# GuidoManni/BodySLAM

Hardware: AMD Instinct MI355X
Metric: frames/sec depth+pose+back-proj, 640x480 seq (higher is better)
Workload: dtype f16

## Files before the change

### bodyslam_amd/_lib.py

```python
from __future__ import annotations

import ctypes as C
import os
from typing import Optional

import torch

_HERE = os.path.dirname(os.path.abspath(__file__))
LIB_PATH = os.environ.get("BODYSLAM_HIP_LIB") or os.path.join(_HERE, "libbodyslam_hip.so")

F32, F16, BF16 = 0, 1, 2
F64 = 3
ACT_NONE, ACT_RELU, ACT_GELU, ACT_SOFTPLUS, ACT_SOFTPLUS_FAST = 0, 1, 2, 3, 4
OUT_PLAIN, OUT_SHUFFLE, OUT_QKV = 0, 1, 2

_TORCH2BS = {torch.float32: F32, torch.float16: F16, torch.bfloat16: BF16}
BS2TORCH = {F32: torch.float32, F16: torch.float16, BF16: torch.bfloat16}


class BodySlamHipError(RuntimeError):
    pass


class GemmDesc(C.Structure):
# ... 476 lines not shown
def cast(x, out):
    check(load_library().bs_cast(p(x), p(out), x.numel(), dt(out), stream_ptr()), "bs_cast")


def cast_split(x, out, rows, cols, f8=False):
    check(load_library().bs_cast_split(p(x), p(out), rows, cols, dt(out) | (32 if f8 else 0), stream_ptr()), "bs_cast_split")


def relu_split(x, out, rows, cols, f8=False):
    check(load_library().bs_relu_split(p(x), p(out), rows, cols, dt(out) | (32 if f8 else 0), stream_ptr()), "bs_relu_split")


def preprocess_patches(frames, out, B, H, W, nh, nw, flip):
    check(load_library().bs_preprocess_patches(p(frames), p(out), B, H, W, nh, nw, int(flip), dt(out), stream_ptr()),
          "bs_preprocess_patches")


def preprocess_image(frames, out, B, H, W, nh, nw, flip):
    check(load_library().bs_preprocess_image(p(frames), p(out), B, H, W, nh, nw, int(flip), stream_ptr()), "bs_preprocess_image")


def fill_rows(x, v, B, rows_per_image, cols):
    check(load_library().bs_fill_rows(p(x), p(v), B, rows_per_image, cols, stream_ptr()), "bs_fill_rows")


def resize_bilinear_nhwc(x, out, B, Hin, Win, Cch, Hout, Wout, align_corners=True, split=False):
    check(load_library().bs_resize_bilinear_nhwc(p(x), p(out), B, Hin, Win, Cch, Hout, Wout, int(align_corners) | (4 if split == 2 else (2 if split else 0)), dt(x),
                                                 stream_ptr()), "bs_resize_bilinear_nhwc")


def depth_u16_to_m(depth_u16: torch.Tensor, depth_scale: float, depth_trunc: float) -> torch.Tensor:
    assert depth_u16.dtype == torch.int16 and depth_u16.is_cuda and depth_u16.is_contiguous()
    out = torch.empty(depth_u16.shape, dtype=torch.float32, device=depth_u16.device)
    check(load_library().bs_depth_u16_to_m(p(depth_u16), depth_u16.numel(), float(depth_scale), float(depth_trunc), p(out), stream_ptr()),
          "bs_depth_u16_to_m")
    return out


def col_mean(A, lda, row0, rows_per_group, groups, row_step, K, out, zero=None):
    assert out.dtype == torch.bfloat16 and (zero is None or zero.dtype == torch.float32)
    check(load_library().bs_col_mean(p(A), lda, row0, rows_per_group, groups, row_step, K, p(out), p(zero), 0 if zero is None else zero.numel(),
                                     dt(A), stream_ptr()), "bs_col_mean")


def rank1_bias(abar, dw, out):
    assert abar.dtype == torch.bfloat16 and dw.dtype == torch.bfloat16 and out.dtype == torch.float32
    G, K = abar.shape
    N = dw.shape[0]
    assert dw.shape[1] == K and tuple(out.shape) == (G, N)
    check(load_library().bs_rank1_bias(p(abar), p(dw), p(out), G, N, K, stream_ptr()), "bs_rank1_bias")


def upconv_tapsum(y, bias, out, B, Hin, Win, Cout, Hout, Wout, align_corners=True, split=False, relu=True):
    check(load_library().bs_upconv_tapsum(p(y), p(bias), p(out), B, Hin, Win, Cout, Hout, Wout,
                                          int(align_corners) | (4 if split == 2 else (2 if split else 0)), int(relu), dt(out), stream_ptr()),
          "bs_upconv_tapsum")


def upconv_fused(x, w, bias, out, B, Hin, Win, Cin, Cout, mode=0, split=0, relu=True, f8_scales=(127, 127, 127, 127)):
    check(load_library().bs_upconv_fused(p(x), p(w), p(bias), p(out), B, Hin, Win, Cin, Cout, 2 * Hin, 2 * Win,
                                         1 | (4 if split == 2 else (2 if split else 0)), int(relu), mode, *[int(v) for v in f8_scales], dt(out),
                                         stream_ptr()), "bs_upconv_fused")


def resize_bias_relu_nhwc(x, bias, out, B, Hin, Win, Cch, Hout, Wout, split=False):
    check(load_library().bs_resize_bias_relu_nhwc(p(x), p(bias), p(out), B, Hin, Win, Cch, Hout, Wout, 1 | (2 if split else 0), dt(out), stream_ptr()),
          "bs_resize_bias_relu_nhwc")


def attractor_step(A, bins_prev, bins_out, route, B, Hp, Wp, H, W, groups, n_bins, n_attr):
    check(load_library().bs_attractor_step(p(A), p(bins_prev), p(bins_out), p(route), B, Hp, Wp, H, W, groups, n_bins, n_attr,
                                           stream_ptr()), "bs_attractor_step")


def mlp2(x, ldx, W1, b1, W2, b2, out, M, K1, N1, N2, act2=ACT_SOFTPLUS_FAST):
    check(load_library().bs_mlp2(p(x), ldx, p(W1), p(b1), p(W2), p(b2), p(out), M, K1, N1, N2, act2, dt(x), stream_ptr()), "bs_mlp2")


def mlp2_add(emb, prev, W1, b1, W2, b2, out, B, Hp, Wp, H, W, K1, N1, N2, act2=ACT_SOFTPLUS_FAST, split=False):
    check(load_library().bs_mlp2_add(p(emb), p(prev), p(W1), p(b1), p(W2), p(b2), p(out), B, Hp, Wp, H, W, K1, N1, N2, act2,
                                     dt(emb) | (16 if split else 0), stream_ptr()), "bs_mlp2_add")


def projector_level(z, b_c1, emb_prev, Wc2, b_c2, We, b_e, x_out, emb_out, eh_out, B, Hl, Wl, H, W, PM, E, NE):
    check(load_library().bs_projector_level(p(z), p(b_c1), p(emb_prev), p(Wc2), p(b_c2), p(We), p(b_e), p(x_out), p(emb_out), p(eh_out), B, Hl, Wl,
                                            H, W, PM, E, NE, dt(z), stream_ptr()), "bs_projector_level")


def add_resized(x, prev, out, B, Hp, Wp, H, W, Cch, split=False):
    check(load_library().bs_add_resized(p(x), p(prev), p(out), B, Hp, Wp, H, W, Cch, dt(x) | (16 if split else 0), stream_ptr()),
          "bs_add_resized")


def logbinom_depth(last, Eh, bins, w0_last, w2, b2, route, depth, B, H, W, He, We, min_temp, max_temp):
    check(load_library().bs_logbinom_depth(p(last), p(Eh), p(bins), p(w0_last), p(w2), p(b2), p(route), p(depth), B, H, W, He, We,
                                           min_temp, max_temp, dt(last), stream_ptr()), "bs_logbinom_depth")


def small_attention(qkv, out, B, S, nheads):
    check(load_library().bs_small_attention(p(qkv), p(out), B, S, nheads, dt(out), stream_ptr()), "bs_small_attention")


def route_argmax(logits, ld, route, B):
    check(load_library().bs_route_argmax(p(logits), ld, p(route), B, stream_ptr()), "bs_route_argmax")


def postprocess_depth(depth_net, depth_m, depth_u16, B, H, W, nh, nw, flip):
    check(load_library().bs_postprocess_depth(p(depth_net), p(depth_m), p(depth_u16), B, H, W, nh, nw, int(flip), stream_ptr()),
          "bs_postprocess_depth")


def cyclepose_im2col(frames, pairs, out, P, H, W):
    check(load_library().bs_cyclepose_im2col(p(frames), p(pairs), p(out), P, H, W, dt(out), stream_ptr()), "bs_cyclepose_im2col")


def instnorm_relu_nhwc(x, out, out_f32, scratch, P, HW, Cch, eps=1e-5):
    check(load_library().bs_instnorm_relu_nhwc(p(x), p(out), p(out_f32), p(scratch), P, HW, Cch, eps, dt(out), stream_ptr()),
          "bs_instnorm_relu_nhwc")


def avgpool_nhwc(x, out, P, HW, Cch):
    check(load_library().bs_avgpool_nhwc(p(x), p(out), P, HW, Cch, stream_ptr()), "bs_avgpool_nhwc")


def cyclepose_head(pooled, x2, w_skip_pool, w_skip_x2, b_skip, w1, b1, w2, b2, pose7, T, scratch, P, HW, Cch):
    check(load_library().bs_cyclepose_head(p(pooled), p(x2), p(w_skip_pool), p(w_skip_x2), p(b_skip), p(w1), p(b1), p(w2), p(b2),
                                           p(pose7), p(T), p(scratch), P, HW, Cch, stream_ptr()), "bs_cyclepose_head")


def backproject(depth_u16, K4, depth_scale, depth_trunc, poses, xyz, idx, count, scratch, B, H, W):
    Karr = (C.c_double * 4)(*[float(v) for v in K4])
    check(load_library().bs_backproject(p(depth_u16), B, H, W, C.cast(Karr, C.c_void_p), float(depth_scale), float(depth_trunc),
                                        p(poses), p(xyz), p(idx), p(count), p(scratch), stream_ptr()), "bs_backproject")


def pose_chain(t_rel, N, g0, g_abs):
    g0arr = None
    if g0 is not None:
        g0arr = C.cast((C.c_double * 16)(*[float(v) for v in g0]), C.c_void_p)
    check(load_library().bs_pose_chain(p(t_rel), N, g0arr, p(g_abs), stream_ptr()), "bs_pose_chain")


def pose_chain_from(t_rel, N, g0_dev, g_abs):
    check(load_library().bs_pose_chain_from(p(t_rel), N, p(g0_dev), p(g_abs), stream_ptr()), "bs_pose_chain_from")


def pixel_to_3d(uvd, K4, out, n):
    Karr = (C.c_double * 4)(*[float(v) for v in K4])
    check(load_library().bs_pixel_to_3d(p(uvd), n, C.cast(Karr, C.c_void_p), p(out), stream_ptr()), "bs_pixel_to_3d")


DEPTH_SCALE_MEDIAN, DEPTH_SCALE_FIXED = 0, 1
DEPTH_METRICS_FIELDS = 16


def depth_metrics(pred, gt, gt_lo, gt_hi, scale, workspace, out):
    B, H, W = pred.shape
    assert tuple(gt.shape) == (B, H, W) and pred.is_contiguous() and gt.is_contiguous()
    assert out.dtype == torch.float64 and tuple(out.shape) == (B, DEPTH_METRICS_FIELDS) and out.is_contiguous()
    mode = DEPTH_SCALE_MEDIAN if scale is None else DEPTH_SCALE_FIXED
    check(load_library().bs_depth_metrics(p(pred), p(gt), B, H, W, float(gt_lo), float(gt_hi), mode, 0.0 if scale is None else float(scale),
                                          p(workspace), workspace.numel() * workspace.element_size(), p(out), stream_ptr()), "bs_depth_metrics")


def depth_metrics_workspace(B: int, H: int, W: int) -> int:
    return int(load_library().bs_depth_metrics_workspace(B, H, W))


TRAJ_EVO, TRAJ_TRAINING = 0, 1
# ... 24 lines not shown
```

### bodyslam_amd/csrc/mlp2.hip

```cpp
#include "common.h"

namespace bs {

constexpr int MLP_BM = 256, MLP_K1 = 128, MLP_N1 = 256, MLP_LDS = 131072;

struct MlpAddGeom {
    const void* prev;
    int Hp, Wp, H, W;
    float sy, sx;
};

template <typename T, int FUSE, int SPLIT>
__global__ __launch_bounds__(512) void mlp2_kernel(const T* __restrict__ x, int ldx, const T* __restrict__ W1, const float* __restrict__ b1,
                                                   const T* __restrict__ W2, const float* __restrict__ b2, float* __restrict__ out, int M, int N2,
                                                   int act2, MlpAddGeom ag) {
    typedef typename T16<T>::v8 v8;
    typedef typename T16<T>::v4 v4;
    extern __shared__ __attribute__((aligned(16))) char smem[];
    const int tid = threadIdx.x, lane = tid & 63;
    const int wave = __builtin_amdgcn_readfirstlane(tid >> 6);
    const int m0 = blockIdx.x * MLP_BM;
    const int frow = lane & 15, fq = lane >> 4;

    {
        const int r8 = lane >> 3, chunk = (lane & 7) ^ r8;
        const bool whole = m0 + MLP_BM <= M;
        const char* xl = reinterpret_cast<const char*>(x + (int64_t)(m0 + r8) * ldx + chunk * 8);
        const char* wl = reinterpret_cast<const char*>(W1 + (int64_t)r8 * MLP_K1 + chunk * 8);
        const int64_t xstep = (int64_t)8 * ldx * 2;
#pragma unroll
        for (int it = 0; it < 4; ++it) {
            const int rg = wave + it * 8;
            const char* xs = xl + rg * xstep;
            if (!whole) {
                int m = m0 + rg * 8 + r8;
                m = m < M ? m : M - 1;
                xs = reinterpret_cast<const char*>(x + (int64_t)m * ldx + chunk * 8);
            }
#pragma unroll
            for (int seg = 0; seg < 2; ++seg) {
                if (!FUSE) glds16(xs + seg * 128, smem + seg * 32768 + rg * 1024);
                glds16(wl + (int64_t)rg * 8 * MLP_K1 * 2 + seg * 128, smem + 65536 + seg * 32768 + rg * 1024);
            }
        }
    }
    if constexpr (FUSE) {
        const T* prev = reinterpret_cast<const T*>(ag.prev);
        constexpr int C = MLP_K1, PS = SPLIT ? 2 : 1;
        auto ld8 = [&](const T* ptr, float (&dst)[8]) {
            const v8 h = *reinterpret_cast<const v8*>(ptr);
#pragma unroll
            for (int e = 0; e < 8; ++e) dst[e] = (float)h[e];
            if (SPLIT) {
                const v8 l = *reinterpret_cast<const v8*>(ptr + C);
#pragma unroll
                for (int e = 0; e < 8; ++e) dst[e] += (float)l[e];
            }
        };
        typedef int i32x4_ __attribute__((ext_vector_type(4)));
        i32x4_* rtab = reinterpret_cast<i32x4_*>(smem + MLP_LDS);
        if (tid < MLP_BM) {
            int m = m0 + tid;
            m = m < M ? m : M - 1;
            const int hw = ag.H * ag.W;
            const int b = m / hw, rem = m - b * hw;
            const int oy = rem / ag.W, ox = rem - oy * ag.W;
            const float fy = ag.sy * (float)oy, fx = ag.sx * (float)ox;
            int y0 = (int)fy, x0 = (int)fx;
            y0 = y0 > ag.Hp - 1 ? ag.Hp - 1 : y0;
            x0 = x0 > ag.Wp - 1 ? ag.Wp - 1 : x0;
            const int y1 = y0 + (y0 < ag.Hp - 1 ? 1 : 0), x1 = x0 + (x0 < ag.Wp - 1 ? 1 : 0);
            const float ly = fy - (float)y0, lx = fx - (float)x0, hy = 1.0f - ly, hx = 1.0f - lx;
            const int pb0 = b * ag.Hp * ag.Wp;
            rtab[2 * tid] = i32x4_{(pb0 + y0 * ag.Wp + x0) * C * PS, (pb0 + y0 * ag.Wp + x1) * C * PS, (pb0 + y1 * ag.Wp + x0) * C * PS,
                                   (pb0 + y1 * ag.Wp + x1) * C * PS};
            rtab[2 * tid + 1] = i32x4_{__float_as_int(hx), __float_as_int(lx), __float_as_int(hy), __float_as_int(ly)};
        }
        __syncthreads();
#pragma unroll 2
        for (int k = 0; k < MLP_BM * 16 / 512; ++k) {
            const int idx = tid + k * 512, r = idx >> 4, c8 = idx & 15;
            int m = m0 + r;
            m = m < M ? m : M - 1;
            const i32x4_ po = rtab[2 * r], pw = rtab[2 * r + 1];
            const float hx = __int_as_float(pw[0]), lx = __int_as_float(pw[1]), hy = __int_as_float(pw[2]), ly = __int_as_float(pw[3]);
            const T* pb = prev + c8 * 8;
            float q00[8], q01[8], q10[8], q11[8], av[8];
            ld8(pb + po[0], q00);
            ld8(pb + po[1], q01);
            ld8(pb + po[2], q10);
            ld8(pb + po[3], q11);
            ld8(x + (int64_t)m * ldx + c8 * 8, av);
            const f32x2_ hx2 = {hx, hx}, lx2 = {lx, lx}, hy2 = {hy, hy}, ly2 = {ly, ly};
            v8 o;
#pragma unroll
            for (int e = 0; e < 8; e += 2) {
                f32x2_ v = bilerp2(f32x2_{q00[e], q00[e + 1]}, f32x2_{q01[e], q01[e + 1]}, f32x2_{q10[e], q10[e + 1]}, f32x2_{q11[e], q11[e + 1]}, hx2, lx2,
                                   hy2, ly2);
                v += f32x2_{av[e], av[e + 1]};
                o[e] = T16<T>::from_f32(v[0]);
                o[e + 1] = T16<T>::from_f32(v[1]);
            }
            *reinterpret_cast<v8*>(smem + (c8 >> 3) * 32768 + r * 128 + (((c8 & 7) ^ (r & 7)) << 4)) = o;
        }
    }
    asm volatile("s_waitcnt vmcnt(0)" ::: "memory");
    __syncthreads();

    const int wr = wave >> 1, wc = wave & 1;
    f32x4 acc1[4][8];
#pragma unroll
    for (int i = 0; i < 4; ++i)
#pragma unroll
        for (int j = 0; j < 8; ++j) acc1[i][j] = f32x4{0.f, 0.f, 0.f, 0.f};
    const int sw = frow & 7;
#pragma unroll
    for (int ks = 0; ks < 4; ++ks) {
        const int seg = ks >> 1, kc = (ks & 1) * 4;
        const int coff = ((kc + fq) ^ sw) << 4;
        v8 xf[4], wf[8];
#pragma unroll
        for (int i = 0; i < 4; ++i) xf[i] = *reinterpret_cast<const v8*>(smem + seg * 32768 + (wr * 64 + i * 16 + frow) * 128 + coff);
#pragma unroll
        for (int j = 0; j < 8; ++j) wf[j] = *reinterpret_cast<const v8*>(smem + 65536 + seg * 32768 + (wc * 128 + j * 16 + frow) * 128 + coff);
#pragma unroll
        for (int i = 0; i < 4; ++i)
#pragma unroll
            for (int j = 0; j < 8; ++j) acc1[i][j] = T16<T>::mfma16(wf[j], xf[i], acc1[i][j]);
    }
    const int NF2 = (N2 + 15) >> 4;
    v8 w2f[2][8];
#pragma unroll
    for (int j = 0; j < 2; ++j)
#pragma unroll
        for (int ks = 0; ks < 8; ++ks) {
            const int n = j * 16 + frow;
            v8 z;
#pragma unroll
            for (int e = 0; e < 8; ++e) z[e] = T16<T>::from_f32(0.f);
            w2f[j][ks] = (j < NF2 && n < N2) ? *reinterpret_cast<const v8*>(W2 + (int64_t)n * MLP_N1 + ks * 32 + fq * 8) : z;
        }
    __syncthreads();
#pragma unroll
    for (int j = 0; j < 8; ++j) {
        const int n = wc * 128 + j * 16 + fq * 4;
        const f32x4 bb = *reinterpret_cast<const f32x4*>(b1 + n);
        const int seg = n >> 6, chunk = (n & 63) >> 3, sub = (n & 7) * 2;
#pragma unroll
        for (int i = 0; i < 4; ++i) {
            const int m = wr * 64 + i * 16 + frow;
            v4 h;
#pragma unroll
            for (int e = 0; e < 4; ++e) h[e] = T16<T>::from_f32(fmaxf(acc1[i][j][e] + bb[e], 0.0f));
            *reinterpret_cast<v4*>(smem + seg * 32768 + m * 128 + ((chunk ^ (m & 7)) << 4) + sub) = h;
        }
    }
    __syncthreads();

    f32x4 acc2[2][2];
#pragma unroll
    for (int i = 0; i < 2; ++i)
#pragma unroll
        for (int j = 0; j < 2; ++j) acc2[i][j] = f32x4{0.f, 0.f, 0.f, 0.f};
#pragma unroll
    for (int ks = 0; ks < 8; ++ks) {
        const int seg = ks >> 1, kc = (ks & 1) * 4;
        const int coff = ((kc + fq) ^ sw) << 4;
        v8 af[2];
#pragma unroll
        for (int i = 0; i < 2; ++i) af[i] = *reinterpret_cast<const v8*>(smem + seg * 32768 + (wave * 32 + i * 16 + frow) * 128 + coff);
#pragma unroll
        for (int i = 0; i < 2; ++i)
#pragma unroll
            for (int j = 0; j < 2; ++j)
                if (j < NF2) acc2[i][j] = T16<T>::mfma16(w2f[j][ks], af[i], acc2[i][j]);
    }
#pragma unroll
    for (int j = 0; j < 2; ++j) {
        const int n = j * 16 + fq * 4;
        if (j >= NF2 || n >= N2) continue;
        const f32x4 bb = *reinterpret_cast<const f32x4*>(b2 + n);
#pragma unroll
        for (int i = 0; i < 2; ++i) {
            const int m = m0 + wave * 32 + i * 16 + frow;
            if (m >= M) continue;
            f32x4 y;
#pragma unroll
            for (int e = 0; e < 4; ++e) y[e] = apply_act(acc2[i][j][e] + bb[e], act2);
            *reinterpret_cast<f32x4*>(out + (int64_t)m * N2 + n) = y;
        }
    }
}

template <typename T, int FUSE, int SPLIT>
static int launch_mlp2(const void* x, int ldx, const void* W1, const float* b1, const void* W2, const float* b2, float* out, int M, int N2, int act2,
                       const MlpAddGeom& ag, hipStream_t st) {
    BS_MAX_DYNAMIC_LDS(((const void*)mlp2_kernel<T, FUSE, SPLIT>), MLP_LDS + (FUSE ? MLP_BM * 32 : 0));
    hipLaunchKernelGGL((mlp2_kernel<T, FUSE, SPLIT>), dim3(cdiv(M, MLP_BM)), dim3(512), MLP_LDS + (FUSE ? MLP_BM * 32 : 0), st, (const T*)x, ldx, (const T*)W1, b1, (const T*)W2, b2,
                       out, M, N2, act2, ag);
    BS_CHECK_LAUNCH();
    return BS_OK;
}

static int mlp2_check(const char* who, const void* x, const void* W1, const float* b1, const void* W2, const float* b2, float* out, int M, int K1,
                      int N1, int N2, int act2, int dtype) {
    if (!initialized()) { set_error("%s: call bs_init first", who); return BS_ERR_NOT_INIT; }
    BS_REQUIRE(x && W1 && b1 && W2 && b2 && out, "%s: null operand", who);
    BS_REQUIRE(dtype == BS_F16 || dtype == BS_BF16, "%s: dtype must be f16 or bf16", who);
    BS_REQUIRE(K1 == MLP_K1 && N1 == MLP_N1, "%s: built for K1 = %d, N1 = %d (got %d, %d)", who, MLP_K1, MLP_N1, K1, N1);
    BS_REQUIRE(N2 > 0 && N2 <= 32 && N2 % 4 == 0, "%s: N2 = %d must be a multiple of 4 in 4 .. 32", who, N2);
    BS_REQUIRE(M > 0, "%s: M = %d", who, M);
    BS_REQUIRE(act2 == BS_ACT_NONE || act2 == BS_ACT_RELU || act2 == BS_ACT_SOFTPLUS || act2 == BS_ACT_SOFTPLUS_FAST || act2 == BS_ACT_GELU, "%s: unknown activation %d", who, act2);
    return BS_OK;
}

}

extern "C" int bs_mlp2(const void* x, int32_t ldx, const void* W1, const float* b1, const void* W2, const float* b2, float* out, int32_t M,
                       int32_t K1, int32_t N1, int32_t N2, int32_t act2, int32_t dtype, void* stream) {
    using namespace bs;
    const int rc = mlp2_check("bs_mlp2", x, W1, b1, W2, b2, out, M, K1, N1, N2, act2, dtype);
    if (rc != BS_OK) return rc;
    BS_REQUIRE(ldx >= K1 && ldx % 8 == 0, "bs_mlp2: ldx = %d (rows of >= K1 16-bit values, 16-byte aligned)", ldx);
    hipStream_t st = (hipStream_t)stream;
    const MlpAddGeom ag{};
    return dtype == BS_F16 ? launch_mlp2<f16, 0, 0>(x, ldx, W1, b1, W2, b2, out, M, N2, act2, ag, st)
                           : launch_mlp2<bf16, 0, 0>(x, ldx, W1, b1, W2, b2, out, M, N2, act2, ag, st);
}

extern "C" int bs_mlp2_add(const void* emb, const void* prev, const void* W1, const float* b1, const void* W2, const float* b2, float* out,
                           int32_t B, int32_t Hp, int32_t Wp, int32_t H, int32_t W, int32_t K1, int32_t N1, int32_t N2, int32_t act2, int32_t dtype,
                           void* stream) {
    using namespace bs;
    const int split = (dtype & 16) ? 1 : 0;
    dtype &= 15;
    BS_REQUIRE(B > 0 && Hp > 0 && Wp > 0 && H > 0 && W > 0 && (int64_t)B * H * W < 0x7FFFFFFFll, "bs_mlp2_add: bad geometry");
    const int M = B * H * W;
    const int rc = mlp2_check("bs_mlp2_add", emb, W1, b1, W2, b2, out, M, K1, N1, N2, act2, dtype);
    if (rc != BS_OK) return rc;
    BS_REQUIRE(prev, "bs_mlp2_add: null operand");
    BS_REQUIRE((int64_t)B * Hp * Wp * K1 * (split ? 2 : 1) < 0x7FFFFFFFll, "bs_mlp2_add: prev too large for 32-bit element offsets");
    MlpAddGeom ag;
    ag.prev = prev; ag.Hp = Hp; ag.Wp = Wp; ag.H = H; ag.W = W;
    ag.sy = H > 1 ? (float)(Hp - 1) / (float)(H - 1) : 0.f;
    ag.sx = W > 1 ? (float)(Wp - 1) / (float)(W - 1) : 0.f;
    const int ldx = K1 * (split ? 2 : 1);
    hipStream_t st = (hipStream_t)stream;
    if (dtype == BS_F16)
        return split ? launch_mlp2<f16, 1, 1>(emb, ldx, W1, b1, W2, b2, out, M, N2, act2, ag, st)
                     : launch_mlp2<f16, 1, 0>(emb, ldx, W1, b1, W2, b2, out, M, N2, act2, ag, st);
    return split ? launch_mlp2<bf16, 1, 1>(emb, ldx, W1, b1, W2, b2, out, M, N2, act2, ag, st)
                 : launch_mlp2<bf16, 1, 0>(emb, ldx, W1, b1, W2, b2, out, M, N2, act2, ag, st);
}
```

### bodyslam_amd/csrc/projector.hip

```cpp
#include "common.h"

namespace bs {

constexpr int PL_PM = 64, PL_E = 128, PL_NE_MAX = 80;
constexpr int PL_WE_OFF = 2 * PL_E * 128;
constexpr int PL_W_BYTES = PL_WE_OFF + 2 * PL_NE_MAX * 128;
constexpr int PL_SLICE = 8192, PL_LDS = PL_W_BYTES + 8 * PL_SLICE;

struct PlArgs {
    const void *z, *prev, *Wc2, *We;
    const float *b1, *bc2, *be;
    void *x_out, *emb_out;
    float* eh_out;
    int B, Hl, Wl, H, W, NE;
    float sy, sx;
    int nslices;
};

#define PL_MFMA_FENCE()                                    \
    do {                                                   \
        __builtin_amdgcn_sched_barrier(0);                 \
        asm volatile("s_nop 15\n\ts_nop 15" ::: "memory"); \
        __builtin_amdgcn_sched_barrier(0);                 \
    } while (0)

template <typename T>
__global__ __launch_bounds__(512) void projector_level_kernel(PlArgs a) {
    typedef typename T16<T>::v8 v8;
    extern __shared__ __attribute__((aligned(16))) char smem[];
    const int tid = threadIdx.x, lane = tid & 63;
    const int wave = __builtin_amdgcn_readfirstlane(tid >> 6);
    const int frow = lane & 15, fq = lane >> 4, sw = frow & 7;
    const int c8 = lane & 7, pq = lane >> 3;
    const int NE = a.NE, nje = NE >> 4;

    {
        const int r8 = lane >> 3, chunk = (lane & 7) ^ r8;
        const int ngc = PL_E / 8, nge = NE / 8, total = 2 * ngc + (a.We ? 2 * nge : 0);
        for (int g = wave; g < total; g += 8) {
            const T* src;
            char* dst;
            if (g < 2 * ngc) {
                const int part = g / ngc, rg = g - part * ngc;
                src = reinterpret_cast<const T*>(a.Wc2) + (int64_t)(rg * 8 + r8) * (3 * PL_PM) + part * (2 * PL_PM) + chunk * 8;
                dst = smem + part * (PL_E * 128) + rg * 1024;
            } else {
                const int g2 = g - 2 * ngc, part = g2 / nge, rg = g2 - part * nge;
                src = reinterpret_cast<const T*>(a.We) + (int64_t)(rg * 8 + r8) * (3 * PL_PM) + part * (2 * PL_PM) + chunk * 8;
                dst = smem + PL_WE_OFF + part * (NE * 128) + rg * 1024;
            }
            glds16(src, dst);
        }
        asm volatile("s_waitcnt vmcnt(0)" ::: "memory");
        __syncthreads();
    }

    char* my = smem + PL_W_BYTES + wave * PL_SLICE;
    const T* zp = reinterpret_cast<const T*>(a.z);
    const T* pp = reinterpret_cast<const T*>(a.prev);
    T* xo = reinterpret_cast<T*>(a.x_out);
    T* eo = reinterpret_cast<T*>(a.emb_out);
    float bz[8];
#pragma unroll
    for (int e = 0; e < 8; ++e) bz[e] = a.b1[c8 * 8 + e];

    auto ld8 = [&](const T* ptr, int lo_off, float (&dst)[8]) {
        const v8 h = *reinterpret_cast<const v8*>(ptr);
        const v8 l = *reinterpret_cast<const v8*>(ptr + lo_off);
#pragma unroll
        for (int e = 0; e < 8; ++e) dst[e] = (float)h[e];
#pragma unroll
        for (int e = 0; e < 8; ++e) dst[e] += (float)l[e];
    };

    for (int s = blockIdx.x * 8 + wave; s < a.nslices; s += gridDim.x * 8) {
        const int m0 = s * 32;
        const int row = m0 / a.W, ox0 = m0 - row * a.W;
        const int b = row / a.H, oy = row - b * a.H;
        const float fy = a.sy * (float)oy;
        int y0 = (int)fy;
        y0 = y0 > a.Hl - 1 ? a.Hl - 1 : y0;
        const int y1 = y0 + (y0 < a.Hl - 1 ? 1 : 0);
        const float ly = fy - (float)y0, hy = 1.0f - ly;
        const f32x2_ hy2 = {hy, hy}, ly2 = {ly, ly};
        const int64_t img = (int64_t)b * a.Hl * a.Wl;
        const int r0 = y0 * a.Wl, r1 = y1 * a.Wl;

        const T* zb = zp + img * (2 * PL_PM) + c8 * 8;
#pragma unroll
        for (int it = 0; it < 4; ++it) {
            const int p = it * 8 + pq, ox = ox0 + p;
            const float fx = a.sx * (float)ox;
            int x0 = (int)fx;
            x0 = x0 > a.Wl - 1 ? a.Wl - 1 : x0;
            const int x1 = x0 + (x0 < a.Wl - 1 ? 1 : 0);
            const float lx = fx - (float)x0, hx = 1.0f - lx;
            float q00[8], q01[8], q10[8], q11[8];
            ld8(zb + (int64_t)(r0 + x0) * (2 * PL_PM), PL_PM, q00);
            ld8(zb + (int64_t)(r0 + x1) * (2 * PL_PM), PL_PM, q01);
            ld8(zb + (int64_t)(r1 + x0) * (2 * PL_PM), PL_PM, q10);
            ld8(zb + (int64_t)(r1 + x1) * (2 * PL_PM), PL_PM, q11);
            const f32x2_ hx2 = {hx, hx}, lx2 = {lx, lx};
            v8 o, ol;
#pragma unroll
            for (int e = 0; e < 8; e += 2) {
                f32x2_ v = bilerp2(f32x2_{q00[e], q00[e + 1]}, f32x2_{q01[e], q01[e + 1]}, f32x2_{q10[e], q10[e + 1]}, f32x2_{q11[e], q11[e + 1]}, hx2, lx2,
                                   hy2, ly2);
                v += f32x2_{bz[e], bz[e + 1]};
                v = f32x2_{fmaxf(v[0], 0.0f), fmaxf(v[1], 0.0f)};
#pragma unroll
                for (int u = 0; u < 2; ++u) {
                    o[e + u] = T16<T>::from_f32(v[u]);
                    ol[e + u] = T16<T>::from_f32(v[u] - (float)o[e + u]);
                }
            }
            const int pos = p * 128 + ((c8 ^ (p & 7)) << 4);
            *reinterpret_cast<v8*>(my + pos) = o;
            *reinterpret_cast<v8*>(my + 4096 + pos) = ol;
        }
        asm volatile("s_waitcnt lgkmcnt(0)" ::: "memory");
        __builtin_amdgcn_wave_barrier();

        if (a.eh_out) {
            f32x4 acc[2][PL_NE_MAX / 16];
#pragma unroll
            for (int i = 0; i < 2; ++i)
#pragma unroll
                for (int j = 0; j < PL_NE_MAX / 16; ++j) acc[i][j] = f32x4{0.f, 0.f, 0.f, 0.f};
#pragma unroll
            for (int pass = 0; pass < 3; ++pass) {
                const int aseg = pass == 1 ? 4096 : 0, wpart = pass == 2 ? NE * 128 : 0;
#pragma unroll
                for (int ks = 0; ks < 2; ++ks) {
                    const int coff = ((ks * 4 + fq) ^ sw) << 4;
                    v8 xf[2];
#pragma unroll
                    for (int i = 0; i < 2; ++i) xf[i] = *reinterpret_cast<const v8*>(my + aseg + (i * 16 + frow) * 128 + coff);
#pragma unroll
                    for (int j = 0; j < PL_NE_MAX / 16; ++j) {
                        if (j < nje) {
                            const v8 wf = *reinterpret_cast<const v8*>(smem + PL_WE_OFF + wpart + (j * 16 + frow) * 128 + coff);
#pragma unroll
                            for (int i = 0; i < 2; ++i) acc[i][j] = T16<T>::mfma16(wf, xf[i], acc[i][j]);
                        }
                    }
                }
            }
            PL_MFMA_FENCE();
#pragma unroll
            for (int j = 0; j < PL_NE_MAX / 16; ++j) {
                if (j < nje) {
                    const int n = j * 16 + fq * 4;
                    const f32x4 bb = *reinterpret_cast<const f32x4*>(a.be + n);
#pragma unroll
                    for (int i = 0; i < 2; ++i) {
                        const f32x4 y = acc[i][j] + bb;
                        *reinterpret_cast<f32x4*>(a.eh_out + (int64_t)(m0 + i * 16 + frow) * NE + n) = y;
                    }
                }
            }
        }

        f32x4 acc[2][8];
#pragma unroll
        for (int i = 0; i < 2; ++i)
#pragma unroll
            for (int j = 0; j < 8; ++j) acc[i][j] = f32x4{0.f, 0.f, 0.f, 0.f};
#pragma unroll
        for (int pass = 0; pass < 3; ++pass) {
            const int aseg = pass == 1 ? 4096 : 0, wpart = pass == 2 ? PL_E * 128 : 0;
#pragma unroll
            for (int ks = 0; ks < 2; ++ks) {
                const int coff = ((ks * 4 + fq) ^ sw) << 4;
                v8 xf[2];
#pragma unroll
                for (int i = 0; i < 2; ++i) xf[i] = *reinterpret_cast<const v8*>(my + aseg + (i * 16 + frow) * 128 + coff);
#pragma unroll
                for (int j = 0; j < 8; ++j) {
                    const v8 wf = *reinterpret_cast<const v8*>(smem + wpart + (j * 16 + frow) * 128 + coff);
#pragma unroll
                    for (int i = 0; i < 2; ++i) acc[i][j] = T16<T>::mfma16(wf, xf[i], acc[i][j]);
                }
            }
        }
        PL_MFMA_FENCE();
        asm volatile("s_waitcnt lgkmcnt(0)" ::: "memory");
        __builtin_amdgcn_wave_barrier();

        const T* pb = pp + img * (2 * PL_E) + c8 * 8;
#pragma unroll
        for (int h = 0; h < 2; ++h) {
#pragma unroll
            for (int jj = 0; jj < 4; ++jj) {
                const f32x4 bb = *reinterpret_cast<const f32x4*>(a.bc2 + h * 64 + jj * 16 + fq * 4);
#pragma unroll
                for (int i = 0; i < 2; ++i) {
                    const int m = i * 16 + frow;
                    *reinterpret_cast<f32x4*>(my + m * 256 + (((jj * 4 + fq) ^ frow) << 4)) = acc[i][h * 4 + jj] + bb;
                }
            }
            asm volatile("s_waitcnt lgkmcnt(0)" ::: "memory");
            __builtin_amdgcn_wave_barrier();
#pragma unroll
            for (int it = 0; it < 4; ++it) {
                const int p = it * 8 + pq, ox = ox0 + p;
                const float fx = a.sx * (float)ox;
                int x0 = (int)fx;
                x0 = x0 > a.Wl - 1 ? a.Wl - 1 : x0;
                const int x1 = x0 + (x0 < a.Wl - 1 ? 1 : 0);
                const float lx = fx - (float)x0, hx = 1.0f - lx;
                float q00[8], q01[8], q10[8], q11[8];
                const T* pc = pb + h * 64;
                ld8(pc + (int64_t)(r0 + x0) * (2 * PL_E), PL_E, q00);
                ld8(pc + (int64_t)(r0 + x1) * (2 * PL_E), PL_E, q01);
                ld8(pc + (int64_t)(r1 + x0) * (2 * PL_E), PL_E, q10);
                ld8(pc + (int64_t)(r1 + x1) * (2 * PL_E), PL_E, q11);
                const f32x4 e0 = *reinterpret_cast<const f32x4*>(my + p * 256 + (((2 * c8) ^ (p & 15)) << 4));
                const f32x4 e1v = *reinterpret_cast<const f32x4*>(my + p * 256 + (((2 * c8 + 1) ^ (p & 15)) << 4));
                const float em[8] = {e0[0], e0[1], e0[2], e0[3], e1v[0], e1v[1], e1v[2], e1v[3]};
                const f32x2_ hx2 = {hx, hx}, lx2 = {lx, lx};
                v8 o;
#pragma unroll
                for (int e = 0; e < 8; e += 2) {
                    f32x2_ v = bilerp2(f32x2_{q00[e], q00[e + 1]}, f32x2_{q01[e], q01[e + 1]}, f32x2_{q10[e], q10[e + 1]}, f32x2_{q11[e], q11[e + 1]}, hx2,
                                       lx2, hy2, ly2);
                    v += f32x2_{em[e], em[e + 1]};
                    o[e] = T16<T>::from_f32(v[0]);
                    o[e + 1] = T16<T>::from_f32(v[1]);
                }
                *reinterpret_cast<v8*>(xo + (int64_t)(m0 + p) * PL_E + h * 64 + c8 * 8) = o;
                if (eo) {
                    v8 eh, el;
#pragma unroll
                    for (int e = 0; e < 8; ++e) {
                        eh[e] = T16<T>::from_f32(em[e]);
                        el[e] = T16<T>::from_f32(em[e] - (float)eh[e]);
                    }
                    T* ep = eo + (int64_t)(m0 + p) * (2 * PL_E) + h * 64 + c8 * 8;
                    *reinterpret_cast<v8*>(ep) = eh;
                    *reinterpret_cast<v8*>(ep + PL_E) = el;
                }
            }
            asm volatile("s_waitcnt lgkmcnt(0)" ::: "memory");
            __builtin_amdgcn_wave_barrier();
        }
    }
}

template <typename T>
static int launch_projector_level(const PlArgs& a, hipStream_t st) {
    BS_MAX_DYNAMIC_LDS(((const void*)projector_level_kernel<T>), PL_LDS);
    const int nblk = cdiv(a.nslices, 8);
    const int grid = nblk < cu_count() ? nblk : cu_count();
    hipLaunchKernelGGL((projector_level_kernel<T>), dim3(grid), dim3(512), PL_LDS, st, a);
    BS_CHECK_LAUNCH();
    return BS_OK;
}

}

extern "C" int bs_projector_level(const void* z, const float* b_c1, const void* emb_prev, const void* Wc2, const float* b_c2, const void* We,
                                  const float* b_e, void* x_out, void* emb_out, float* eh_out, int32_t B, int32_t Hl, int32_t Wl, int32_t H,
                                  int32_t W, int32_t PM, int32_t E, int32_t NE, int32_t dtype, void* stream) {
    using namespace bs;
    if (!initialized()) { set_error("bs_projector_level: call bs_init first"); return BS_ERR_NOT_INIT; }
    BS_REQUIRE(z && b_c1 && emb_prev && Wc2 && b_c2 && x_out, "bs_projector_level: null operand");
    BS_REQUIRE(dtype == BS_F16 || dtype == BS_BF16, "bs_projector_level: dtype must be f16 or bf16");
    BS_REQUIRE(PM == PL_PM && E == PL_E, "bs_projector_level: built for a %d-channel hidden map and a %d-channel embedding (got %d, %d)", PL_PM, PL_E, PM, E);
    BS_REQUIRE((We == nullptr) == (eh_out == nullptr) && (We == nullptr || b_e != nullptr), "bs_projector_level: We, b_e and eh_out go together");
    BS_REQUIRE(We == nullptr || (NE > 0 && NE <= PL_NE_MAX && NE % 16 == 0), "bs_projector_level: NE = %d must be a multiple of 16 up to %d", NE, PL_NE_MAX);
    BS_REQUIRE(B > 0 && Hl > 0 && Wl > 0 && H > 0 && W > 0 && W % 32 == 0, "bs_projector_level: bad geometry (W must be a multiple of 32: a wave takes 32 pixels of one row)");
    BS_REQUIRE((int64_t)B * H * W < 0x7FFFFFFFll && (int64_t)Hl * Wl * 2 * PL_E < 0x7FFFFFFFll, "bs_projector_level: too large for 32-bit pixel indices");
    PlArgs a;
    a.z = z; a.prev = emb_prev; a.Wc2 = Wc2; a.We = We; a.b1 = b_c1; a.bc2 = b_c2; a.be = b_e;
    a.x_out = x_out; a.emb_out = emb_out; a.eh_out = eh_out;
    a.B = B; a.Hl = Hl; a.Wl = Wl; a.H = H; a.W = W; a.NE = We ? NE : 16;
    a.sy = H > 1 ? (float)(Hl - 1) / (float)(H - 1) : 0.f;
    a.sx = W > 1 ? (float)(Wl - 1) / (float)(W - 1) : 0.f;
    a.nslices = (int)((int64_t)B * H * W / 32);
    hipStream_t st = (hipStream_t)stream;
    return dtype == BS_F16 ? launch_projector_level<f16>(a, st) : launch_projector_level<bf16>(a, st);
}
```

Baseline: 476.6.

## Halve MLP tile with staged W1 halves and pair rows in projector bilerp

The fused two-layer MLP kernel now uses 128-row tiles with half the LDS. It stages the first-layer weights in two halves, overlapping their loads with MFMA work, and keeps hidden activations in registers until a single LDS write-back. It also requests 4 waves per EU to raise occupancy. The projector kernel now lets a wave handle 16 pixels from each of two adjacent output rows that share the same source rows, so each horizontal interpolation is reused for both rows, with a flag to turn this off. The risks are more barriers and register pressure in the MLP, and scattered output addressing in paired mode.

```diff
diff --git a/bodyslam_amd/_lib.py b/bodyslam_amd/_lib.py
--- a/bodyslam_amd/_lib.py
+++ b/bodyslam_amd/_lib.py
@@ -582,9 +582,9 @@
                                      dt(emb) | (16 if split else 0), stream_ptr()), "bs_mlp2_add")
 
 
-def projector_level(z, b_c1, emb_prev, Wc2, b_c2, We, b_e, x_out, emb_out, eh_out, B, Hl, Wl, H, W, PM, E, NE):
+def projector_level(z, b_c1, emb_prev, Wc2, b_c2, We, b_e, x_out, emb_out, eh_out, B, Hl, Wl, H, W, PM, E, NE, single_rows=False):
     check(load_library().bs_projector_level(p(z), p(b_c1), p(emb_prev), p(Wc2), p(b_c2), p(We), p(b_e), p(x_out), p(emb_out), p(eh_out), B, Hl, Wl,
-                                            H, W, PM, E, NE, dt(z), stream_ptr()), "bs_projector_level")
+                                            H, W, PM, E, NE, dt(z) | (16 if single_rows else 0), stream_ptr()), "bs_projector_level")
 
 
 def add_resized(x, prev, out, B, Hp, Wp, H, W, Cch, split=False):
diff --git a/bodyslam_amd/csrc/mlp2.hip b/bodyslam_amd/csrc/mlp2.hip
--- a/bodyslam_amd/csrc/mlp2.hip
+++ b/bodyslam_amd/csrc/mlp2.hip
@@ -2,7 +2,8 @@
 
 namespace bs {
 
-constexpr int MLP_BM = 256, MLP_K1 = 128, MLP_N1 = 256, MLP_LDS = 131072;
+constexpr int MLP_BM = 128, MLP_K1 = 128, MLP_N1 = 256, MLP_LDS = 65536;
+constexpr int MLP_SEG = MLP_BM * 128, MLP_W_OFF = 2 * MLP_SEG;
 
 struct MlpAddGeom {
     const void* prev;
@@ -11,7 +12,7 @@
 };
 
 template <typename T, int FUSE, int SPLIT>
-__global__ __launch_bounds__(512) void mlp2_kernel(const T* __restrict__ x, int ldx, const T* __restrict__ W1, const float* __restrict__ b1,
+__global__ __launch_bounds__(512) __attribute__((amdgpu_waves_per_eu(4, 4))) void mlp2_kernel(const T* __restrict__ x, int ldx, const T* __restrict__ W1, const float* __restrict__ b1,
                                                    const T* __restrict__ W2, const float* __restrict__ b2, float* __restrict__ out, int M, int N2,
                                                    int act2, MlpAddGeom ag) {
     typedef typename T16<T>::v8 v8;
@@ -21,28 +22,43 @@
     const int wave = __builtin_amdgcn_readfirstlane(tid >> 6);
     const int m0 = blockIdx.x * MLP_BM;
     const int frow = lane & 15, fq = lane >> 4;
-
+    const int wr = wave >> 1, wc = wave & 1;
+    f32x4 bb1[4];
+    auto load_b1 = [&](int half) {
+#pragma unroll
+        for (int j = 0; j < 4; ++j) bb1[j] = *reinterpret_cast<const f32x4*>(b1 + half * 128 + wc * 64 + j * 16 + fq * 4);
+    };
+
+    const int r8 = lane >> 3, chunk = (lane & 7) ^ r8;
+    const char* wl = reinterpret_cast<const char*>(W1 + (int64_t)r8 * MLP_K1 + chunk * 8);
+    auto stage_w1 = [&](int half, int seg) {
+#pragma unroll
+        for (int it = 0; it < 2; ++it) {
+            const int rg = wave + it * 8;
+            glds16(wl + (int64_t)(half * 128 + rg * 8) * MLP_K1 * 2 + seg * 128, smem + MLP_W_OFF + seg * MLP_SEG + rg * 1024);
+        }
+    };
     {
-        const int r8 = lane >> 3, chunk = (lane & 7) ^ r8;
         const bool whole = m0 + MLP_BM <= M;
         const char* xl = reinterpret_cast<const char*>(x + (int64_t)(m0 + r8) * ldx + chunk * 8);
-        const char* wl = reinterpret_cast<const char*>(W1 + (int64_t)r8 * MLP_K1 + chunk * 8);
         const int64_t xstep = (int64_t)8 * ldx * 2;
-#pragma unroll
-        for (int it = 0; it < 4; ++it) {
-            const int rg = wave + it * 8;
-            const char* xs = xl + rg * xstep;
-            if (!whole) {
-                int m = m0 + rg * 8 + r8;
-                m = m < M ? m : M - 1;
-                xs = reinterpret_cast<const char*>(x + (int64_t)m * ldx + chunk * 8);
+        if (!FUSE) {
+#pragma unroll
+            for (int it = 0; it < 2; ++it) {
+                const int rg = wave + it * 8;
+                const char* xs = xl + rg * xstep;
+                if (!whole) {
+                    int m = m0 + rg * 8 + r8;
+                    m = m < M ? m : M - 1;
+                    xs = reinterpret_cast<const char*>(x + (int64_t)m * ldx + chunk * 8);
+                }
+#pragma unroll
+                for (int seg = 0; seg < 2; ++seg) glds16(xs + seg * 128, smem + seg * MLP_SEG + rg * 1024);
             }
-#pragma unroll
-            for (int seg = 0; seg < 2; ++seg) {
-                if (!FUSE) glds16(xs + seg * 128, smem + seg * 32768 + rg * 1024);
-                glds16(wl + (int64_t)rg * 8 * MLP_K1 * 2 + seg * 128, smem + 65536 + seg * 32768 + rg * 1024);
-            }
-        }
+        }
+        stage_w1(0, 0);
+        stage_w1(0, 1);
+        load_b1(0);
     }
     if constexpr (FUSE) {
         const T* prev = reinterpret_cast<const T*>(ag.prev);
@@ -101,94 +117,126 @@
                 o[e] = T16<T>::from_f32(v[0]);
                 o[e + 1] = T16<T>::from_f32(v[1]);
             }
-            *reinterpret_cast<v8*>(smem + (c8 >> 3) * 32768 + r * 128 + (((c8 & 7) ^ (r & 7)) << 4)) = o;
+            *reinterpret_cast<v8*>(smem + (c8 >> 3) * MLP_SEG + r * 128 + (((c8 & 7) ^ (r & 7)) << 4)) = o;
         }
     }
     asm volatile("s_waitcnt vmcnt(0)" ::: "memory");
     __syncthreads();
 
-    const int wr = wave >> 1, wc = wave & 1;
-    f32x4 acc1[4][8];
-#pragma unroll
-    for (int i = 0; i < 4; ++i)
-#pragma unroll
-        for (int j = 0; j < 8; ++j) acc1[i][j] = f32x4{0.f, 0.f, 0.f, 0.f};
     const int sw = frow & 7;
-#pragma unroll
-    for (int ks = 0; ks < 4; ++ks) {
-        const int seg = ks >> 1, kc = (ks & 1) * 4;
-        const int coff = ((kc + fq) ^ sw) << 4;
-        v8 xf[4], wf[8];
-#pragma unroll
-        for (int i = 0; i < 4; ++i) xf[i] = *reinterpret_cast<const v8*>(smem + seg * 32768 + (wr * 64 + i * 16 + frow) * 128 + coff);
-#pragma unroll
-        for (int j = 0; j < 8; ++j) wf[j] = *reinterpret_cast<const v8*>(smem + 65536 + seg * 32768 + (wc * 128 + j * 16 + frow) * 128 + coff);
-#pragma unroll
-        for (int i = 0; i < 4; ++i)
-#pragma unroll
-            for (int j = 0; j < 8; ++j) acc1[i][j] = T16<T>::mfma16(wf[j], xf[i], acc1[i][j]);
-    }
+    f32x4 acc1[2][4];
+    v4 hid[2][2][4];
+    auto product1 = [&](int seg) {
+#pragma unroll
+        for (int kk = 0; kk < 2; ++kk) {
+            const int coff = ((kk * 4 + fq) ^ sw) << 4;
+            v8 xf[2], wf[4];
+#pragma unroll
+            for (int i = 0; i < 2; ++i) xf[i] = *reinterpret_cast<const v8*>(smem + seg * MLP_SEG + (wr * 32 + i * 16 + frow) * 128 + coff);
+#pragma unroll
+            for (int j = 0; j < 4; ++j) wf[j] = *reinterpret_cast<const v8*>(smem + MLP_W_OFF + seg * MLP_SEG + (wc * 64 + j * 16 + frow) * 128 + coff);
+#pragma unroll
+            for (int i = 0; i < 2; ++i)
+#pragma unroll
+                for (int j = 0; j < 4; ++j) acc1[i][j] = T16<T>::mfma16(wf[j], xf[i], acc1[i][j]);
+        }
+    };
+    auto zero_acc = [&]() {
+#pragma unroll
+        for (int i = 0; i < 2; ++i)
+#pragma unroll
+            for (int j = 0; j < 4; ++j) acc1[i][j] = f32x4{0.f, 0.f, 0.f, 0.f};
+    };
+    auto round_hidden = [&](int half) {
+#pragma unroll
+        for (int j = 0; j < 4; ++j)
+#pragma unroll
+            for (int i = 0; i < 2; ++i)
+#pragma unroll
+                for (int e = 0; e < 4; ++e) hid[half][i][j][e] = T16<T>::from_f32(fmaxf(acc1[i][j][e] + bb1[j][e], 0.0f));
+#pragma unroll
+        for (int i = 0; i < 2; ++i)
+#pragma unroll
+            for (int j = 0; j < 4; ++j) asm volatile("" : "+v"(hid[half][i][j])::"memory");
+    };
+    auto bare_barrier = [&]() {
+        __builtin_amdgcn_sched_barrier(0);
+        __builtin_amdgcn_s_barrier();
+        __builtin_amdgcn_sched_barrier(0);
+        asm volatile("" ::: "memory");
+    };
+    zero_acc();
+    product1(0);
+    __syncthreads();
+    stage_w1(1, 0);
+    product1(1);
+    bare_barrier();
+    stage_w1(1, 1);
+    round_hidden(0);
+    zero_acc();
+    asm volatile("s_waitcnt vmcnt(2)" ::: "memory");
+    bare_barrier();
+    product1(0);
+    asm volatile("s_waitcnt vmcnt(0)" ::: "memory");
+    __syncthreads();
+    load_b1(1);
+    product1(1);
+    round_hidden(1);
     const int NF2 = (N2 + 15) >> 4;
-    v8 w2f[2][8];
-#pragma unroll
-    for (int j = 0; j < 2; ++j)
+    v8 w2f[8];
+    f32x4 bb2;
+    auto load_w2 = [&](int j) {
+        const int nb = j * 16 + fq * 4;
+        bb2 = *reinterpret_cast<const f32x4*>(b2 + (nb < N2 ? nb : 0));
 #pragma unroll
         for (int ks = 0; ks < 8; ++ks) {
             const int n = j * 16 + frow;
             v8 z;
 #pragma unroll
             for (int e = 0; e < 8; ++e) z[e] = T16<T>::from_f32(0.f);
-            w2f[j][ks] = (j < NF2 && n < N2) ? *reinterpret_cast<const v8*>(W2 + (int64_t)n * MLP_N1 + ks * 32 + fq * 8) : z;
-        }
-    __syncthreads();
-#pragma unroll
-    for (int j = 0; j < 8; ++j) {
-        const int n = wc * 128 + j * 16 + fq * 4;
-        const f32x4 bb = *reinterpret_cast<const f32x4*>(b1 + n);
-        const int seg = n >> 6, chunk = (n & 63) >> 3, sub = (n & 7) * 2;
-#pragma unroll
-        for (int i = 0; i < 4; ++i) {
-            const int m = wr * 64 + i * 16 + frow;
-            v4 h;
-#pragma unroll
-            for (int e = 0; e < 4; ++e) h[e] = T16<T>::from_f32(fmaxf(acc1[i][j][e] + bb[e], 0.0f));
-            *reinterpret_cast<v4*>(smem + seg * 32768 + m * 128 + ((chunk ^ (m & 7)) << 4) + sub) = h;
-        }
-    }
-    __syncthreads();
-
-    f32x4 acc2[2][2];
-#pragma unroll
-    for (int i = 0; i < 2; ++i)
-#pragma unroll
-        for (int j = 0; j < 2; ++j) acc2[i][j] = f32x4{0.f, 0.f, 0.f, 0.f};
-#pragma unroll
-    for (int ks = 0; ks < 8; ++ks) {
-        const int seg = ks >> 1, kc = (ks & 1) * 4;
-        const int coff = ((kc + fq) ^ sw) << 4;
-        v8 af[2];
-#pragma unroll
-        for (int i = 0; i < 2; ++i) af[i] = *reinterpret_cast<const v8*>(smem + seg * 32768 + (wave * 32 + i * 16 + frow) * 128 + coff);
-#pragma unroll
-        for (int i = 0; i < 2; ++i)
-#pragma unroll
-            for (int j = 0; j < 2; ++j)
-                if (j < NF2) acc2[i][j] = T16<T>::mfma16(w2f[j][ks], af[i], acc2[i][j]);
-    }
-#pragma unroll
-    for (int j = 0; j < 2; ++j) {
+            const v8 w = *reinterpret_cast<const v8*>(W2 + (int64_t)(n < N2 ? n : N2 - 1) * MLP_N1 + ks * 32 + fq * 8);
+            w2f[ks] = n < N2 ? w : z;
+        }
+    };
+    load_w2(0);
+    __builtin_amdgcn_sched_barrier(0);
+    __syncthreads();
+#pragma unroll
+    for (int half = 0; half < 2; ++half)
+#pragma unroll
+        for (int j = 0; j < 4; ++j) {
+            const int n = half * 128 + wc * 64 + j * 16 + fq * 4;
+            const int seg = n >> 6, chunk = (n & 63) >> 3, sub = (n & 7) * 2;
+#pragma unroll
+            for (int i = 0; i < 2; ++i) {
+                const int m = wr * 32 + i * 16 + frow;
+                *reinterpret_cast<v4*>(smem + seg * MLP_SEG + m * 128 + ((chunk ^ (m & 7)) << 4) + sub) = hid[half][i][j];
+            }
+        }
+    __syncthreads();
+
+    const int m = m0 + wave * 16 + frow;
+    auto product2 = [&](int j) {
+        f32x4 acc2 = f32x4{0.f, 0.f, 0.f, 0.f};
+#pragma unroll
+        for (int ks = 0; ks < 8; ++ks) {
+            const int seg = ks >> 1, kc = (ks & 1) * 4;
+            const int coff = ((kc + fq) ^ sw) << 4;
+            const v8 af = *reinterpret_cast<const v8*>(smem + seg * MLP_SEG + (wave * 16 + frow) * 128 + coff);
+            acc2 = T16<T>::mfma16(w2f[ks], af, acc2);
+        }
         const int n = j * 16 + fq * 4;
-        if (j >= NF2 || n >= N2) continue;
-        const f32x4 bb = *reinterpret_cast<const f32x4*>(b2 + n);
-#pragma unroll
-        for (int i = 0; i < 2; ++i) {
-            const int m = m0 + wave * 32 + i * 16 + frow;
-            if (m >= M) continue;
+        if (n < N2 && m < M) {
             f32x4 y;
 #pragma unroll
-            for (int e = 0; e < 4; ++e) y[e] = apply_act(acc2[i][j][e] + bb[e], act2);
+            for (int e = 0; e < 4; ++e) y[e] = apply_act(acc2[e] + bb2[e], act2);
             *reinterpret_cast<f32x4*>(out + (int64_t)m * N2 + n) = y;
         }
+    };
+    product2(0);
+    if (NF2 > 1) {
+        load_w2(1);
+        product2(1);
     }
 }
 
diff --git a/bodyslam_amd/csrc/projector.hip b/bodyslam_amd/csrc/projector.hip
--- a/bodyslam_amd/csrc/projector.hip
+++ b/bodyslam_amd/csrc/projector.hip
@@ -14,7 +14,7 @@
     float* eh_out;
     int B, Hl, Wl, H, W, NE;
     float sy, sx;
-    int nslices;
+    int nslices, pairs;
 };
 
 #define PL_MFMA_FENCE()                                    \
@@ -72,40 +72,66 @@
 #pragma unroll
         for (int e = 0; e < 8; ++e) dst[e] += (float)l[e];
     };
+    auto xlerp = [&](const T* base, int r0, int r1, int ld, int lo_off, int ox, f32x2_ (&top)[4], f32x2_ (&bot)[4]) {
+        const float fx = a.sx * (float)ox;
+        int x0 = (int)fx;
+        x0 = x0 > a.Wl - 1 ? a.Wl - 1 : x0;
+        const int x1 = x0 + (x0 < a.Wl - 1 ? 1 : 0);
+        const float lx = fx - (float)x0, hx = 1.0f - lx;
+        float q00[8], q01[8], q10[8], q11[8];
+        ld8(base + (int64_t)(r0 + x0) * ld, lo_off, q00);
+        ld8(base + (int64_t)(r0 + x1) * ld, lo_off, q01);
+        ld8(base + (int64_t)(r1 + x0) * ld, lo_off, q10);
+        ld8(base + (int64_t)(r1 + x1) * ld, lo_off, q11);
+        const f32x2_ hx2 = {hx, hx}, lx2 = {lx, lx};
+#pragma unroll
+        for (int e = 0; e < 4; ++e) {
+            top[e] = __builtin_elementwise_fma(lx2, f32x2_{q01[2 * e], q01[2 * e + 1]}, hx2 * f32x2_{q00[2 * e], q00[2 * e + 1]});
+            bot[e] = __builtin_elementwise_fma(lx2, f32x2_{q11[2 * e], q11[2 * e + 1]}, hx2 * f32x2_{q10[2 * e], q10[2 * e + 1]});
+        }
+    };
+    auto ycoef = [&](int oy, int& y0, int& y1, float& ly) {
+        const float fy = a.sy * (float)oy;
+        y0 = (int)fy;
+        y0 = y0 > a.Hl - 1 ? a.Hl - 1 : y0;
+        y1 = y0 + (y0 < a.Hl - 1 ? 1 : 0);
+        ly = fy - (float)y0;
+    };
 
     for (int s = blockIdx.x * 8 + wave; s < a.nslices; s += gridDim.x * 8) {
         const int m0 = s * 32;
-        const int row = m0 / a.W, ox0 = m0 - row * a.W;
+        const int row = m0 / a.W, oxs = m0 - row * a.W;
         const int b = row / a.H, oy = row - b * a.H;
-        const float fy = a.sy * (float)oy;
-        int y0 = (int)fy;
-        y0 = y0 > a.Hl - 1 ? a.Hl - 1 : y0;
-        const int y1 = y0 + (y0 < a.Hl - 1 ? 1 : 0);
-        const float ly = fy - (float)y0, hy = 1.0f - ly;
-        const f32x2_ hy2 = {hy, hy}, ly2 = {ly, ly};
+        int y0, y1;
+        float lyA, lyB = 0.f;
+        ycoef(oy, y0, y1, lyA);
+        bool pair = false;
+        int mA = m0, ox0 = oxs, rs = 16;
+        const int rA = ((oy - 1) & ~1) + 1;
+        if (a.pairs && oy >= 1 && rA + 1 < a.H) {
+            int y0a, y1a, y0b, y1b;
+            float la, lb;
+            ycoef(rA, y0a, y1a, la);
+            ycoef(rA + 1, y0b, y1b, lb);
+            if (y0a == y0b && y1a == y1b) {
+                pair = true;
+                ox0 = ((oy - rA) * (a.W >> 5) + (oxs >> 5)) * 16;
+                mA = (b * a.H + rA) * a.W + ox0;
+                rs = a.W;
+                y0 = y0a; y1 = y1a; lyA = la; lyB = lb;
+            }
+        }
+        const float hyA = 1.0f - lyA, hyB = 1.0f - lyB;
+        const f32x2_ hyA2 = {hyA, hyA}, lyA2 = {lyA, lyA}, hyB2 = {hyB, hyB}, lyB2 = {lyB, lyB};
         const int64_t img = (int64_t)b * a.Hl * a.Wl;
         const int r0 = y0 * a.Wl, r1 = y1 * a.Wl;
 
         const T* zb = zp + img * (2 * PL_PM) + c8 * 8;
-#pragma unroll
-        for (int it = 0; it < 4; ++it) {
-            const int p = it * 8 + pq, ox = ox0 + p;
-            const float fx = a.sx * (float)ox;
-            int x0 = (int)fx;
-            x0 = x0 > a.Wl - 1 ? a.Wl - 1 : x0;
-            const int x1 = x0 + (x0 < a.Wl - 1 ? 1 : 0);
-            const float lx = fx - (float)x0, hx = 1.0f - lx;
-            float q00[8], q01[8], q10[8], q11[8];
-            ld8(zb + (int64_t)(r0 + x0) * (2 * PL_PM), PL_PM, q00);
-            ld8(zb + (int64_t)(r0 + x1) * (2 * PL_PM), PL_PM, q01);
-            ld8(zb + (int64_t)(r1 + x0) * (2 * PL_PM), PL_PM, q10);
-            ld8(zb + (int64_t)(r1 + x1) * (2 * PL_PM), PL_PM, q11);
-            const f32x2_ hx2 = {hx, hx}, lx2 = {lx, lx};
+        auto put_e1 = [&](int p, const f32x2_ (&top)[4], const f32x2_ (&bot)[4], f32x2_ hy2, f32x2_ ly2) {
             v8 o, ol;
 #pragma unroll
             for (int e = 0; e < 8; e += 2) {
-                f32x2_ v = bilerp2(f32x2_{q00[e], q00[e + 1]}, f32x2_{q01[e], q01[e + 1]}, f32x2_{q10[e], q10[e + 1]}, f32x2_{q11[e], q11[e + 1]}, hx2, lx2,
-                                   hy2, ly2);
+                f32x2_ v = __builtin_elementwise_fma(ly2, bot[e >> 1], hy2 * top[e >> 1]);
                 v += f32x2_{bz[e], bz[e + 1]};
                 v = f32x2_{fmaxf(v[0], 0.0f), fmaxf(v[1], 0.0f)};
 #pragma unroll
@@ -117,6 +143,24 @@
             const int pos = p * 128 + ((c8 ^ (p & 7)) << 4);
             *reinterpret_cast<v8*>(my + pos) = o;
             *reinterpret_cast<v8*>(my + 4096 + pos) = ol;
+        };
+        if (pair) {
+#pragma unroll
+            for (int it = 0; it < 2; ++it) {
+                const int p = it * 8 + pq;
+                f32x2_ top[4], bot[4];
+                xlerp(zb, r0, r1, 2 * PL_PM, PL_PM, ox0 + p, top, bot);
+                put_e1(p, top, bot, hyA2, lyA2);
+                put_e1(p + 16, top, bot, hyB2, lyB2);
+            }
+        } else {
+#pragma unroll
+            for (int it = 0; it < 4; ++it) {
+                const int p = it * 8 + pq;
+                f32x2_ top[4], bot[4];
+                xlerp(zb, r0, r1, 2 * PL_PM, PL_PM, ox0 + p, top, bot);
+                put_e1(p, top, bot, hyA2, lyA2);
+            }
         }
         asm volatile("s_waitcnt lgkmcnt(0)" ::: "memory");
         __builtin_amdgcn_wave_barrier();
@@ -155,7 +199,7 @@
 #pragma unroll
                     for (int i = 0; i < 2; ++i) {
                         const f32x4 y = acc[i][j] + bb;
-                        *reinterpret_cast<f32x4*>(a.eh_out + (int64_t)(m0 + i * 16 + frow) * NE + n) = y;
+                        *reinterpret_cast<f32x4*>(a.eh_out + (int64_t)(mA + i * rs + frow) * NE + n) = y;
                     }
                 }
             }
@@ -201,34 +245,21 @@
             }
             asm volatile("s_waitcnt lgkmcnt(0)" ::: "memory");
             __builtin_amdgcn_wave_barrier();
-#pragma unroll
-            for (int it = 0; it < 4; ++it) {
-                const int p = it * 8 + pq, ox = ox0 + p;
-                const float fx = a.sx * (float)ox;
-                int x0 = (int)fx;
-                x0 = x0 > a.Wl - 1 ? a.Wl - 1 : x0;
-                const int x1 = x0 + (x0 < a.Wl - 1 ? 1 : 0);
-                const float lx = fx - (float)x0, hx = 1.0f - lx;
-                float q00[8], q01[8], q10[8], q11[8];
-                const T* pc = pb + h * 64;
-                ld8(pc + (int64_t)(r0 + x0) * (2 * PL_E), PL_E, q00);
-                ld8(pc + (int64_t)(r0 + x1) * (2 * PL_E), PL_E, q01);
-                ld8(pc + (int64_t)(r1 + x0) * (2 * PL_E), PL_E, q10);
-                ld8(pc + (int64_t)(r1 + x1) * (2 * PL_E), PL_E, q11);
+            const T* pc = pb + h * 64;
+            auto put_x = [&](int p, const f32x2_ (&top)[4], const f32x2_ (&bot)[4], f32x2_ hy2, f32x2_ ly2) {
                 const f32x4 e0 = *reinterpret_cast<const f32x4*>(my + p * 256 + (((2 * c8) ^ (p & 15)) << 4));
                 const f32x4 e1v = *reinterpret_cast<const f32x4*>(my + p * 256 + (((2 * c8 + 1) ^ (p & 15)) << 4));
                 const float em[8] = {e0[0], e0[1], e0[2], e0[3], e1v[0], e1v[1], e1v[2], e1v[3]};
-                const f32x2_ hx2 = {hx, hx}, lx2 = {lx, lx};
+                const int64_t m = mA + (p >> 4) * rs + (p & 15);
                 v8 o;
 #pragma unroll
                 for (int e = 0; e < 8; e += 2) {
-                    f32x2_ v = bilerp2(f32x2_{q00[e], q00[e + 1]}, f32x2_{q01[e], q01[e + 1]}, f32x2_{q10[e], q10[e + 1]}, f32x2_{q11[e], q11[e + 1]}, hx2,
-                                       lx2, hy2, ly2);
+                    f32x2_ v = __builtin_elementwise_fma(ly2, bot[e >> 1], hy2 * top[e >> 1]);
                     v += f32x2_{em[e], em[e + 1]};
                     o[e] = T16<T>::from_f32(v[0]);
                     o[e + 1] = T16<T>::from_f32(v[1]);
                 }
-                *reinterpret_cast<v8*>(xo + (int64_t)(m0 + p) * PL_E + h * 64 + c8 * 8) = o;
+                *reinterpret_cast<v8*>(xo + m * PL_E + h * 64 + c8 * 8) = o;
                 if (eo) {
                     v8 eh, el;
 #pragma unroll
@@ -236,9 +267,27 @@
                         eh[e] = T16<T>::from_f32(em[e]);
                         el[e] = T16<T>::from_f32(em[e] - (float)eh[e]);
                     }
-                    T* ep = eo + (int64_t)(m0 + p) * (2 * PL_E) + h * 64 + c8 * 8;
+                    T* ep = eo + m * (2 * PL_E) + h * 64 + c8 * 8;
                     *reinterpret_cast<v8*>(ep) = eh;
                     *reinterpret_cast<v8*>(ep + PL_E) = el;
+                }
+            };
+            if (pair) {
+#pragma unroll
+                for (int it = 0; it < 2; ++it) {
+                    const int p = it * 8 + pq;
+                    f32x2_ top[4], bot[4];
+                    xlerp(pc, r0, r1, 2 * PL_E, PL_E, ox0 + p, top, bot);
+                    put_x(p, top, bot, hyA2, lyA2);
+                    put_x(p + 16, top, bot, hyB2, lyB2);
+                }
+            } else {
+#pragma unroll
+                for (int it = 0; it < 4; ++it) {
+                    const int p = it * 8 + pq;
+                    f32x2_ top[4], bot[4];
+                    xlerp(pc, r0, r1, 2 * PL_E, PL_E, ox0 + p, top, bot);
+                    put_x(p, top, bot, hyA2, lyA2);
                 }
             }
             asm volatile("s_waitcnt lgkmcnt(0)" ::: "memory");
@@ -263,6 +312,8 @@
                                   const float* b_e, void* x_out, void* emb_out, float* eh_out, int32_t B, int32_t Hl, int32_t Wl, int32_t H,
                                   int32_t W, int32_t PM, int32_t E, int32_t NE, int32_t dtype, void* stream) {
     using namespace bs;
+    const int pairs = (dtype & 16) ? 0 : 1;
+    dtype &= 15;
     if (!initialized()) { set_error("bs_projector_level: call bs_init first"); return BS_ERR_NOT_INIT; }
     BS_REQUIRE(z && b_c1 && emb_prev && Wc2 && b_c2 && x_out, "bs_projector_level: null operand");
     BS_REQUIRE(dtype == BS_F16 || dtype == BS_BF16, "bs_projector_level: dtype must be f16 or bf16");
@@ -278,6 +329,7 @@
     a.sy = H > 1 ? (float)(Hl - 1) / (float)(H - 1) : 0.f;
     a.sx = W > 1 ? (float)(Wl - 1) / (float)(W - 1) : 0.f;
     a.nslices = (int)((int64_t)B * H * W / 32);
+    a.pairs = pairs;
     hipStream_t st = (hipStream_t)stream;
     return dtype == BS_F16 ? launch_projector_level<f16>(a, st) : launch_projector_level<bf16>(a, st);
 }
```

After: 477.0, median of 4. About the same (+0.1%).
